# SIA-IDE/MMGT

Hardware: AMD Instinct MI355X
Metric: UNet3D denoise-steps/sec at 512x512x24 bf16 (higher is better)
Workload: dtype bf16; 1 GPU; BASELINE configs[1]: 512x512x24 pose2vid denoise step (CFG batch 2, UNet3D + MM-HAA, 16 reference banks, 1 window of 24 frames, guidance 3.5, DDIM v-pred), random-init weights; frames=24, parallelism=clip-parallel x1

## Files before the change

mmgt_amd/csrc/gemm.hip:

```cpp
#include <string.h>

#include <type_traits>

#include "common.h"
#include "gemm_common.h"
#include "mmgt_hip.h"

#ifndef MMGT_GEMM_VARIANT
#define MMGT_GEMM_VARIANT 7
#endif

namespace {

constexpr bool V_FRAGDB = (MMGT_GEMM_VARIANT & 1) != 0;
constexpr bool V_ILV = (MMGT_GEMM_VARIANT & 2) != 0;
constexpr bool V_LATE = (MMGT_GEMM_VARIANT & 4) != 0;
constexpr bool V_LATE_ALL = (MMGT_GEMM_VARIANT & 8) != 0;
constexpr bool V_NODMA = (MMGT_GEMM_VARIANT & 16) != 0;

template <int CTRL>
__device__ __forceinline__ unsigned dpp_quad(unsigned v) {
  return (unsigned)__builtin_amdgcn_mov_dpp((int)v, CTRL, 0xf, 0xf, true);
}
template <int S>
// ... 526 lines not shown
            }
          }
        };
        using std::integral_constant;
        group(integral_constant<int, 0>{}, integral_constant<int, (TN >= 2 ? 2 : 1)>{});
        if constexpr (TN > 2) group(integral_constant<int, 2>{}, integral_constant<int, (TN >= 4 ? 2 : 1)>{});
        if constexpr (TN > 4) group(integral_constant<int, 4>{}, integral_constant<int, (TN >= 6 ? 2 : 1)>{});
      }
    } else if (FULL_OK) {
#pragma unroll
      for (int i = 0; i < TM; ++i) {
        const int m = row0 + 32 * i + lr;
        if (m >= M) continue;
#pragma unroll
        for (int j = 0; j < TN; ++j) {
          if (geglu && (j & 1)) continue;
#pragma unroll
          for (int r = 0; r < 16; ++r) {
            const int nl = acc_row(r, lane);
            const int ncol = col0 + 32 * j + nl;
            if (ncol >= N) continue;
            float x = acc[i][j][r];
            if (ep.bias) x += ep.bias[ncol];
            long ocol = ncol;
            if (geglu) {
              float gte = acc[i][(j + 1) < TN ? j + 1 : j][r];
              if (ep.bias) gte += ep.bias[ncol + 32];
              x *= gelu_erf_f(gte);
              ocol = (long)((col0 + 32 * j) >> 1) + nl;
            } else {
              if (ep.bias2) x += ep.bias2[(long)(m / ep.bias2_rows) * N + ncol];
              if (ep.act == 2) x = silu_f(x);
              if (ep.act == 3) x = fmaxf(x, 0.f);
              if (ep.act == 4) x = quick_gelu_f(x);
              if (ep.act == 5) x = gelu_erf_f(x);
              if (ep.act == 6) x = mish_f(x);
              x *= (ep.row_scale ? ep.row_scale[m] : 1.f) * ep.alpha;
              if (POST_OK && ep.bias_post) x += ep.bias_post[ncol];
            }
            if (res) x += Elem<T>::ld(res + (long)m * ep.ldr + ocol);
            Elem<T>::st(out + (long)m * ep.ldo + ocol, x);
          }
        }
      }
    }
  }
}

template <typename T, int MODE, int BM, int BN, int WM, int WN, int NSTAGE, int ROWB = 128, int EPI = 0>
int launch_cfg(const ADesc& ad, const void* W, long bsw, const Epi& ep, int M, int N, int K, int batch, hipStream_t s) {
  const int tiles_m = (M + BM - 1) / BM, tiles_n = (N + BN - 1) / BN;
  const size_t lds = (size_t)NSTAGE * (BM + BN) * ROWB;
  auto kern = gemm_kernel<T, MODE, BM, BN, WM, WN, NSTAGE, ROWB, EPI>;
  static int resident = 0;
  if (!resident) {
    if (hipFuncSetAttribute(reinterpret_cast<const void*>(kern), hipFuncAttributeMaxDynamicSharedMemorySize, (int)lds) !=
        hipSuccess) {
      mmgt_set_error("gemm: cannot reserve %zu bytes of LDS", lds);
      return 2;
    }
    int per_cu = 0, dev = 0;
    hipDeviceProp_t prop;
    if (hipOccupancyMaxActiveBlocksPerMultiprocessor(&per_cu, kern, WM * WN * 64, lds) != hipSuccess || per_cu < 1 ||
        hipGetDevice(&dev) != hipSuccess || hipGetDeviceProperties(&prop, dev) != hipSuccess) {
      mmgt_set_error("gemm: occupancy query failed");
      return 2;
    }
    resident = per_cu * prop.multiProcessorCount;
  }
  long gx = (resident + batch - 1) / batch;
  gx = (gx + 7) / 8 * 8;
  if (gx > (long)tiles_m * tiles_n) gx = (long)tiles_m * tiles_n;
  dim3 grid((unsigned)gx, 1, batch);
  hipLaunchKernelGGL(kern, grid, dim3(WM * WN * 64), lds, s, ad, reinterpret_cast<const char*>(W), bsw, ep, M, N, K, tiles_m,
                     tiles_n);
  MMGT_LAUNCH_CHECK();
  return 0;
}

int g_splitk = 1;
int g_tailsplit = 1;
int g_gemm_cfg = 0;
int g_bm192 = 1;

}
int mmgt_gemm16_launch(int mode, int bn, const void* ad, const void* W, long bsw, const void* ep, int M, int N, int K,
                       int batch, void* stream);
int mmgt_gemm16_splitk(int mode, int bn, const void* ad, const void* W, const void* ep, int M, int N, int K, int S, void* stream, int m0);
namespace {

template <typename T, int MODE>
int launch(const ADesc& ad, const void* W, long bsw, const Epi& ep, int M, int N, int K, int batch, hipStream_t s) {
  const bool geglu = ep.act == 1;
  int cfg = g_gemm_cfg;
  if ((cfg == 0 || cfg == 18) && g_splitk && std::is_same<T, bf16_t>::value && batch == 1 && ep.act == 0 && ep.fast && !ep.row_scale &&
      ep.alpha == 1.f && !ep.bias_post && N % 8 == 0 && K >= 2560 && (N % 256 == 0 || N % 320 == 0) &&
      (((uintptr_t)ep.bias | (uintptr_t)ep.bias2) & 15) == 0) {
    const int bn = N % 256 == 0 ? 256 : 320;
    const long tiles = (long)((M + 255) / 256) * (N / bn);
    const int nch = K / 64;
    int S = 0;
    for (int c = 8; c >= 2; --c)
      if (tiles * c <= 256 && nch % c == 0 && nch / c >= (tiles <= 64 ? 16 : 64)) { S = c; break; }
    if (S >= 2 && tiles <= 128 && (MODE == 1 || tiles <= 32 || tiles > 64)) return mmgt_gemm16_splitk(MODE, bn, &ad, W, &ep, M, N, K, S, s, 0);
  }
  if (cfg == 18) cfg = 0;
  if (cfg == 0) {
    const long tiles128 = (long)((M + 127) / 128) * ((N + 127) / 128) * batch;
    const long tiles256 = (long)((M + 255) / 256) * ((N + 127) / 128) * batch;
    const long tiles256sq = (long)((M + 255) / 256) * ((N + 255) / 256) * batch;
    const bool big_ok = N % 256 == 0 && K >= 2560 && tiles256sq >= 192 && tiles256sq <= 512;
    const bool sq_ok = ((N + 255) / 256) * 256l * 100 <= (long)N * 107 && ((M + 255) / 256) * 256l * 100 <= (long)M * 115 && tiles256sq >= 192;
    const bool b16 = std::is_same<T, bf16_t>::value;
    if (MODE == 1) {
      if (b16 && N % 320 == 0 && (M >= 49152 || (M >= 24576 && N >= 640))) cfg = 17;
      else if (b16 && N % 256 == 0 && tiles256sq >= 192) cfg = 16;
      else cfg = (N % 320 == 0 && M >= 49152) ? 12 : big_ok ? 9 : (tiles128 < 512 || N <= 64) ? 3 : 1;
    } else if (b16 && !geglu && N % 320 == 0 && N <= 960 && M >= 131072) cfg = 17;
    else if (b16 && !geglu && N % 320 == 0 && N <= 1280 && M >= 49152 && (K >= 1280 || ep.residual || N == 1280)) cfg = 17;
    else if (b16 && !geglu && N == 640 && M >= 24576 && K >= 2560 && g_bm192) cfg = 17;
    else if (sq_ok) cfg = b16 ? 16 : 9;
    else if (geglu || K >= 1280) cfg = tiles256 >= 256 ? 6 : (!geglu && tiles128 <= 256) ? 3 : 1;
    else if (M >= 131072 && N >= 640) cfg = 6;
    else cfg = 1;
  }
  if (geglu && (cfg == 3 || cfg == 12)) cfg = 1;
  if (MODE == 1 && ad.up >= 2 && cfg != 16 && cfg != 17) cfg = N % 320 == 0 ? 17 : 16;
  bool bm192 = cfg == 19;
  if (cfg == 19) cfg = 17;
  if (cfg == 17 && !bm192 && g_gemm_cfg == 0 && g_bm192 && std::is_same<T, bf16_t>::value && batch == 1 && N % 320 == 0) {
    const long tn = N / 320;
    const long r256 = (((long)(M + 255) / 256) * tn + 255) / 256, r192 = (((long)(M + 191) / 192) * tn + 255) / 256;
    bm192 = (double)r192 * 0.88 < (double)r256 * 0.97;
  }
  if (cfg == 16 || cfg == 17) {
    const bool post = ep.row_scale || ep.alpha != 1.f || ep.bias_post;
    if (std::is_same<T, bf16_t>::value && ep.fast && ep.act <= (cfg == 16 && !post ? 1 : 0) &&
        (((uintptr_t)ep.bias | (uintptr_t)ep.bias2 | (uintptr_t)ep.bias_post) & 15) == 0 && N % 4 == 0) {
      const int bn = cfg == 16 ? 256 : bm192 ? 192320 : 320;
      const int bnc = cfg == 16 ? 256 : 320;
      const long tiles_n = (N + bnc - 1) / bnc, tiles_m = (M + 255) / 256, ntile = tiles_m * tiles_n;
      const int nch = K / 64;
      if (g_tailsplit && (!bm192 || g_gemm_cfg == 0) && MODE == 1 && batch == 1 && !ad.ksplit && ep.act == 0 && !post && N % bnc == 0 && N % 8 == 0 && K >= 2560 && nch % 2 == 0 && ntile > 256) {
        const long rows_a = (256 * (ntile / 256) / tiles_n) * 256;
        const long tail = (tiles_m - rows_a / 256) * tiles_n;
        const long img = MODE == 1 ? (long)ad.OH * ad.OW : 1;
        if (rows_a > 0 && rows_a < M && tail > 0 && 2 * tail <= 256 && 4 * tail >= 256 && rows_a % img == 0) {
          int rc = mmgt_gemm16_launch(MODE, bnc, &ad, W, bsw, &ep, (int)rows_a, N, K, 1, s);
          if (rc) return rc;
          ADesc adb = ad;
          Epi epb = ep;
          const long esz = sizeof(T);
          if (MODE == 1) {
            const long n0 = rows_a / img;
            adb.src0 = ad.src0 + n0 * ad.IH * ad.IW * ad.C0 * esz;
            if (ad.src1) adb.src1 = ad.src1 + n0 * ad.IH * ad.IW * ad.C1 * esz;
          } else {
            adb.src0 = ad.src0 + rows_a * ad.ld0 * esz;
          }
          if (ep.residual) epb.residual = ep.residual + rows_a * ep.ldr * esz;
          epb.out = ep.out + rows_a * ep.ldo * esz;
          return mmgt_gemm16_splitk(MODE, bnc, &adb, W, &epb, (int)(M - rows_a), N, K, 2, s, (int)rows_a);
        }
      }
      return mmgt_gemm16_launch(MODE, bn, &ad, W, bsw, &ep, M, N, K, batch, s);
    }
    if (MODE == 1 && ad.up >= 2) {
      mmgt_set_error("conv: the four-phase upsample form and the two-source 1 x 1 conv need the gemm16 path (bf16, 16-byte aligned bias, Cout %% 4 == 0)");
      return 1;
    }
    cfg = cfg == 16 ? 9 : geglu ? 1 : 12;
  }
  if (cfg == 20) {
    if (std::is_same<T, bf16_t>::value && ep.fast && ep.act == 0 && (((uintptr_t)ep.bias | (uintptr_t)ep.bias2 | (uintptr_t)ep.bias_post) & 15) == 0 && N % 4 == 0)
      return mmgt_gemm16_launch(MODE, 128, &ad, W, bsw, &ep, M, N, K, batch, s);
    cfg = 1;
  }
  if (!ep.fast || ep.act >= 2) return launch_cfg<T, MODE, 128, 128, 2, 2, 2, 128, 2>(ad, W, bsw, ep, M, N, K, batch, s);
  if (ep.row_scale || ep.alpha != 1.f || ep.bias_post) {
    if (MODE == 0 && !geglu) return launch_cfg<T, 0, 128, 128, 2, 2, 2, 128, 1>(ad, W, bsw, ep, M, N, K, batch, s);
    return launch_cfg<T, MODE, 128, 128, 2, 2, 2, 128, 2>(ad, W, bsw, ep, M, N, K, batch, s);
  }
#ifdef MMGT_GEMM_AB
  switch (cfg) {
    case 3: return launch_cfg<T, MODE, 128, 64, 2, 2, 2>(ad, W, bsw, ep, M, N, K, batch, s);
    case 6: return launch_cfg<T, MODE, 256, 128, 4, 2, 3>(ad, W, bsw, ep, M, N, K, batch, s);
    case 9: return launch_cfg<T, MODE, 256, 256, 2, 4, 2>(ad, W, bsw, ep, M, N, K, batch, s);
    case 12: return launch_cfg<T, MODE, 128, 320, 4, 2, 2>(ad, W, bsw, ep, M, N, K, batch, s);
    default: return launch_cfg<T, MODE, 128, 128, 2, 2, 2>(ad, W, bsw, ep, M, N, K, batch, s);
  }
#else
  switch (cfg) {
    case 1: return launch_cfg<T, MODE, 128, 128, 2, 2, 2>(ad, W, bsw, ep, M, N, K, batch, s);
    case 3: return launch_cfg<T, MODE, 128, 64, 2, 2, 2>(ad, W, bsw, ep, M, N, K, batch, s);
    case 6: return launch_cfg<T, MODE, 256, 128, 4, 2, 3>(ad, W, bsw, ep, M, N, K, batch, s);
    case 9: return launch_cfg<T, MODE, 256, 256, 2, 4, 2>(ad, W, bsw, ep, M, N, K, batch, s);
    case 12: return launch_cfg<T, MODE, 128, 320, 4, 2, 2>(ad, W, bsw, ep, M, N, K, batch, s);
    default: return launch_cfg<T, MODE, 128, 128, 2, 2, 2>(ad, W, bsw, ep, M, N, K, batch, s);
  }
#endif
}

int epi_fast(const Epi& ep, int N, int n_out, int esz) {
  auto al16 = [](const void* p) { return (reinterpret_cast<uintptr_t>(p) & 15) == 0; };
  bool ok = N % 8 == 0 && n_out % 8 == 0 && al16(ep.out) && (ep.ldo * esz) % 16 == 0 && (ep.bso * esz) % 16 == 0;
  ok = ok && (ep.bias2 == nullptr || ep.bias2_rows >= 256);
  if (ep.residual) ok = ok && al16(ep.residual) && (ep.ldr * esz) % 16 == 0 && (ep.bsr * esz) % 16 == 0;
  return ok ? 1 : 0;
}

int check_common(int dtype, int M, int N, int K, int act) {
  MMGT_CHECK(dtype == MMGT_F32 || dtype == MMGT_BF16, "gemm: bad dtype %d", dtype);
  MMGT_CHECK(M > 0 && N > 0 && K > 0, "gemm: empty problem M=%d N=%d K=%d", M, N, K);
  MMGT_CHECK(K % 64 == 0, "gemm: K=%d must be a multiple of 64 (pad channels on the host)", K);
  MMGT_CHECK(act >= 0 && act <= 6, "gemm: bad act %d", act);
  MMGT_CHECK(act != 1 || N % 64 == 0, "gemm: GEGLU needs N %% 64 == 0 (N=%d)", N);
  return 0;
}

}

void mmgt_attn_set64(int v);
void mmgt_gn_set_rows(int v);
void mmgt_attn_set_heads_inner(int v);
void mmgt_attn_set_attn80(int v);
void mmgt_attn_set_nomax(int v);
void mmgt_gemm16_set_pb(int v);
void mmgt_gemm16_set_stagger(int v);
void mmgt_gn_set_interleave(int v);
void mmgt_gn_set_lpr0(int v);
void mmgt_gn_set_narrow(int v);
void mmgt_gn_set_slab(int v);
void mmgt_ffn_set_dbg(int v);
void mmgt_rowgemm_set_dbg(int v);
void mmgt_tleg_set_abl(int v);
void mmgt_gnconv_set_abl(int v);
void mmgt_rconv_set_abl(int v);
void mmgt_rconv_set_stagger(int v);
void mmgt_rconv_set_cb(int v);
namespace {
struct HostSwitch { const char* key; int value; };
HostSwitch g_host[] = {
    {"fused_ff", 1},
    {"twin_attention", 1},
    {"shared_rows", 1},
    {"oz3", 1},
    {"rowgemm", 1},
    {"tleg", 1},
    {"rconv", 5},
    {"conv_out_taps", 1},
    {"ffpo_cat", 1},
    {"sc_cat", 1},
    {"up2", 1},
    {"rconv_stats", 1},
    {"gnconv", 2},
    {"zero_audio_skip", 1},
    {"window_state", 1},
    {"smga_graph", 1},
};
}
extern "C" int mmgt_tune_get(const char* key, int* value) {
  if (key && value)
    for (const HostSwitch& h : g_host)
      if (!strcmp(key, h.key)) { *value = h.value; return 0; }
  mmgt_set_error("tune_get: unknown key");
  return 1;
}
extern "C" int mmgt_tune(const char* key, int value) {
  if (key)
    for (HostSwitch& h : g_host)
      if (!strcmp(key, h.key)) { h.value = value; return 0; }
  if (key && !strcmp(key, "gemm_cfg")) { g_gemm_cfg = value; return 0; }
  if (key && !strcmp(key, "attn64")) { mmgt_attn_set64(value); return 0; }
  if (key && !strcmp(key, "attn_nomax") && (value == 0 || value == 1)) { mmgt_attn_set_nomax(value); return 0; }
  if (key && !strcmp(key, "attn_heads_inner")) { mmgt_attn_set_heads_inner(value); return 0; }
  if (key && !strcmp(key, "attn80")) { mmgt_attn_set_attn80(value); return 0; }
  if (key && !strcmp(key, "g16_pb")) { mmgt_gemm16_set_pb(value); return 0; }
  if (key && !strcmp(key, "g16_stagger")) { mmgt_gemm16_set_stagger(value); return 0; }
  if (key && !strcmp(key, "gn_rows")) { mmgt_gn_set_rows(value); return 0; }
  if (key && !strcmp(key, "gn_interleave")) { mmgt_gn_set_interleave(value); return 0; }
  if (key && !strcmp(key, "gn_narrow")) { mmgt_gn_set_narrow(value); return 0; }
  if (key && !strcmp(key, "gn_slab")) { mmgt_gn_set_slab(value); return 0; }
  if (key && !strcmp(key, "gn_lpr0")) { if (value != 4 && value != 8 && value != 16) return -1; mmgt_gn_set_lpr0(value); return 0; }
  if (key && !strcmp(key, "splitk")) { g_splitk = value; return 0; }
  if (key && !strcmp(key, "bm192")) { g_bm192 = value; return 0; }
  if (key && !strcmp(key, "tailsplit")) { g_tailsplit = value; return 0; }
  if (key && !strcmp(key, "rconv_cb") && (value == 0 || value == 320 || value == 256 || value == 160)) { mmgt_rconv_set_cb(value); return 0; }
  if (key && !strcmp(key, "rconv_stagger") && value >= 0 && value <= 8192) { mmgt_rconv_set_stagger(value); return 0; }
#ifdef MMGT_ABLATE
  if (key && !strcmp(key, "ffn_dbg") && value >= 0 && value <= 2) { mmgt_ffn_set_dbg(value); return 0; }
  if (key && !strcmp(key, "gnconv_abl") && value >= 0 && value <= 255) { mmgt_gnconv_set_abl(value); return 0; }
  if (key && !strcmp(key, "tleg_abl") && value >= 0 && value <= 128) { mmgt_tleg_set_abl(value); return 0; }
  if (key && !strcmp(key, "rconv_abl") && value >= 0 && value <= 31) { mmgt_rconv_set_abl(value); return 0; }
  if (key && !strcmp(key, "rowgemm_dbg") && value >= 0 && value <= 5) { mmgt_rowgemm_set_dbg(value); return 0; }
#else
  if (key && !strcmp(key, "rowgemm_dbg") && (value == 0 || value == 5)) { mmgt_rowgemm_set_dbg(value); return 0; }
  if (key && (!strcmp(key, "ffn_dbg") || !strcmp(key, "gnconv_abl") || !strcmp(key, "tleg_abl") || !strcmp(key, "rconv_abl") || !strcmp(key, "rowgemm_dbg"))) {
    mmgt_set_error("tune: '%s' selects a timing ablation whose results are garbage; the product library does not contain them (build libmmgt_hip_abl.so with `make -C mmgt_amd/csrc abl` and load it through MMGT_LIB)", key);
    return 1;
  }
#endif
  mmgt_set_error("tune: unknown key");
  return 1;
}

namespace {
template <typename T>
__global__ __launch_bounds__(256) void gemv_kernel(const T* __restrict__ A, long lda, const T* __restrict__ W, const float* __restrict__ bias,
                                                   T* __restrict__ out, long ldo, int M, int N, int K, int act) {
  constexpr int VEC = 16 / sizeof(T);
  const int lane = threadIdx.x & 63, n = blockIdx.x * 4 + (threadIdx.x >> 6);
  if (n >= N) return;
  float acc[4] = {0.f, 0.f, 0.f, 0.f};
  const T* w = W + (long)n * K;
  for (int k = lane * VEC; k < K; k += 64 * VEC) {
    union { u32x4 u; T e[VEC]; } wv, av;
    wv.u = *reinterpret_cast<const u32x4*>(w + k);
#pragma unroll
    for (int m = 0; m < 4; ++m)
      if (m < M) {
        av.u = *reinterpret_cast<const u32x4*>(A + m * lda + k);
#pragma unroll
        for (int e = 0; e < VEC; ++e) acc[m] = fmaf(Elem<T>::ld(&wv.e[e]), Elem<T>::ld(&av.e[e]), acc[m]);
      }
  }
#pragma unroll
  for (int m = 0; m < 4; ++m) {
    float v = acc[m];
    for (int o = 32; o > 0; o >>= 1) v += __shfl_xor(v, o);
    if (lane == 0 && m < M) {
      v += bias ? bias[n] : 0.f;
      if (act == 2) v = silu_f(v);
      Elem<T>::st(out + m * ldo + n, v);
    }
  }
}
}

static int gemm_entry(const void* A, long lda, const void* W, const float* bias, const float* bias2, int bias2_rows,
                      const float* row_scale, float alpha, const float* bias_post, const void* residual, long ldr, void* out,
                      long ldo, int M, int N, int K, int act, int batch, long bsA, long bsW, long bsR, long bsO, int dtype,
                      void* stream) {
  if (check_common(dtype, M, N, K, act)) return 1;
  MMGT_CHECK(A && W && out, "gemm: null pointer");
  MMGT_CHECK(lda >= 1 && batch >= 1, "gemm: lda %ld < 1 or batch %d < 1", lda, batch);
  MMGT_CHECK(!bias2 || bias2_rows > 0, "gemm: bias2_rows must be positive");
  const int esz = dtype == MMGT_BF16 ? 2 : 4;
  MMGT_CHECK(((uintptr_t)A % 16) == 0 && ((uintptr_t)W % 16) == 0 && (lda * esz) % 16 == 0 && (bsA * esz) % 16 == 0 &&
                 (bsW * esz) % 16 == 0,
             "gemm: A/W must be 16-byte aligned with 16-byte aligned rows");
  MMGT_CHECK(((long)(M - 1) * lda + K) * esz < (1l << 31) && (long)N * K * esz < (1l << 31),
             "gemm: an operand (per batch entry) exceeds the 2 GiB range of the 32-bit LDS-DMA offsets");
  if (M == 1 && batch == 1 && !bias2 && !row_scale && alpha == 1.f && !bias_post && !residual && (act == 0 || act == 2) && K % (16 / esz) == 0) {
    if (dtype == MMGT_BF16)
      hipLaunchKernelGGL(gemv_kernel<bf16_t>, dim3((unsigned)((N + 3) / 4)), dim3(256), 0, (hipStream_t)stream, (const bf16_t*)A, lda, (const bf16_t*)W, bias,
                         (bf16_t*)out, ldo, M, N, K, act);
    else
      hipLaunchKernelGGL(gemv_kernel<float>, dim3((unsigned)((N + 3) / 4)), dim3(256), 0, (hipStream_t)stream, (const float*)A, lda, (const float*)W, bias,
                         (float*)out, ldo, M, N, K, act);
    MMGT_LAUNCH_CHECK();
    return 0;
  }
  ADesc ad{};
  ad.src0 = (const char*)A;
  ad.ld0 = lda;
  ad.bs0 = bsA;
  Epi ep{};
  ep.bias = bias; ep.bias2 = bias2; ep.bias2_rows = bias2_rows; ep.row_scale = row_scale; ep.alpha = alpha;
// ... 89 lines not shown
```

mmgt_amd/csrc/gemm16.hip:

```cpp
#include <type_traits>

#include "common.h"
#include "gemm_common.h"
#include "mmgt_hip.h"

namespace {

typedef __attribute__((ext_vector_type(4))) float acc4;

__device__ __forceinline__ acc4 mma16(s16x8 a, s16x8 b, acc4 c) {
  return __builtin_amdgcn_mfma_f32_16x16x32_bf16(a, b, c, 0, 0, 0);
}

template <int MODE, int BN, int BM = 256>
__global__ __launch_bounds__(512, 2) void gemm16_kernel(ADesc ad, const char* __restrict__ W, long bsw, Epi ep, int M, int N,
                                                        int K, int tiles_m, int tiles_n, int pb_stg, unsigned long long* trace) {
  extern __shared__ __attribute__((aligned(1024))) char smem[];
  typedef bf16_t T;
  static_assert(BN == 128 || BN == 256 || BN == 320, "BN");
  static_assert(BM == 256 || BM == 192, "BM");
  constexpr int ESZ = 2, ROWB = 128, BK = 64, NW = 8;
  constexpr int WROWS = BM / 4, RT = WROWS / 16;
  constexpr int A_BYTES = BM * ROWB, B_BYTES = BN * ROWB, STAGE_BYTES = A_BYTES + B_BYTES;
  constexpr int CPR = 8, RPD = 8;
  constexpr int GA = BM / RPD / NW, GB = BN / RPD / NW;
  constexpr int NPH = BN / 64, NT = BN / 32;
  constexpr int BIAS_OFF = 2 * STAGE_BYTES, BIAS_ARR = 2048, NBP = BN == 320 ? 2 : 1;
  auto swz = [](int row) { return (row >> 1) & 7; };

  const int nwg = tiles_m * tiles_n;
  const int pb = pb_stg & 255, stg = pb_stg >> 8;
  const int bz = blockIdx.z;
  const int tid = threadIdx.x, lane = tid & 63, wid = __builtin_amdgcn_readfirstlane(tid >> 6);
  const int wr = wid >> 2;
  const int wm = wid >> 1, wn = wid & 1;
  const int lm = lane & 15, lq = lane >> 4;
  int trace_n = 0;
  auto stamp = [&](int k) {
    if (trace && (wid & 3) == 0 && lane == 0 && trace_n < 32) trace[(((long)blockIdx.x * 32 + trace_n) * 2 + wr) * 4 + k] = wall_clock64();
  };

  auto decode = [&](int v, int& tm, int& tn) {
    const int q = nwg >> 3, r = nwg & 7, x = v & 7;
    const int t = (x < r ? x * (q + 1) : r * (q + 1) + (x - r) * q) + (v >> 3);
    if (pb <= 1) {
      tm = t / tiles_n;
      tn = t - tm * tiles_n;
    } else {
      const int gsz = pb * tiles_n, g = t / gsz, w = t - g * gsz;
      const int pbe = min(pb, tiles_m - g * pb);
      tn = w / pbe;
      tm = g * pb + (w - tn * pbe);
    }
  };

  const int srow = lane / CPR, spos = lane % CPR;
  const int ldw = ad.ksplit ? ad.ldw : K;
  const long kstart = ad.ksplit ? (long)bz * K : 0;
  const T* a0 = reinterpret_cast<const T*>(ad.src0) + (ad.ksplit ? (MODE == 0 ? kstart : 0) : (long)bz * ad.bs0);
  const T* a1 = ad.src1 ? reinterpret_cast<const T*>(ad.src1) + (ad.ksplit ? 0 : (long)bz * ad.bs1) : nullptr;
  const T* wbase = reinterpret_cast<const T*>(W) + (ad.ksplit ? kstart : (long)bz * bsw);
  const __amdgpu_buffer_rsrc_t rA0 = dma_rsrc(a0), rA1 = dma_rsrc(a1 ? a1 : a0), rW = dma_rsrc(wbase);
  const int c0sw = spos ^ (srow >> 1);
  int limA = 0, limW = 0;
  unsigned aoff[MODE == 0 ? 2 : GA];
  unsigned woff[2];
  unsigned am0 = 0;
  int a_step = 0, w_step = 0;
  int p_tap = 0, p_c = 0, a_soff = 0;
  bool a_second = false, a_fresh = true;
  auto setupA = [&](int tm) {
    const unsigned row = (unsigned)(tm * BM + wid * GA * RPD + srow);
    if (MODE == 0) {
      a_step = (int)(RPD * ad.ld0 * ESZ);
      limA = M - (int)row;
#pragma unroll
      for (int q = 0; q < 2; ++q) aoff[q] = row * (unsigned)(ad.ld0 * ESZ) + (unsigned)((c0sw ^ (4 * ((q + wid * GA) & 1))) << 4);
    } else {
      am0 = row;
    }
    p_tap = MODE == 1 ? (int)(kstart / (ad.C0 + ad.C1)) : 0;
    p_c = MODE == 1 ? (int)(kstart - (long)p_tap * (ad.C0 + ad.C1)) : 0;
    a_fresh = true;
  };
  auto setupW = [&](int tn) {
    const unsigned row = (unsigned)(tn * BN + wid * GB * RPD + srow);
    w_step = RPD * ldw * ESZ;
    limW = N - (int)row;
#pragma unroll
    for (int q = 0; q < 2; ++q) woff[q] = row * (unsigned)(ldw * ESZ) + (unsigned)((c0sw ^ (4 * ((q + wid * GB) & 1))) << 4);
  };
  auto prepA = [&](int ch) {
    if (MODE == 0) {
      a_soff = ch * ROWB;
    } else {
      const int cin = ad.C0 + ad.C1;
      if (p_c == 0 || p_c == ad.C0 || a_fresh) {
        a_fresh = false;
        const bool up2 = ad.up == 2;
        const int ky = up2 ? p_tap >> 1 : ad.up == 3 ? 1 : p_tap / 3, kx = up2 ? p_tap & 1 : ad.up == 3 ? 1 : p_tap - ky * 3;
        const int vh = ad.up == 1 ? ad.IH * 2 : ad.IH, vw = ad.up == 1 ? ad.IW * 2 : ad.IW;
        const bool second = p_c >= ad.C0 && ad.C1 > 0;
        const unsigned cpb = (unsigned)(second ? ad.C1 : ad.C0) * ESZ;
        a_second = second;
        a_soff = (p_c - (second ? ad.C0 : 0)) * ESZ;
// ... 135 lines not shown
        int m = row0 + 16 * i + lm;
        if (m >= M) m = M - 1;
        second[i] = ep.bias2 && m / b2div != b2r0;
      }
#pragma unroll
      for (int j = 0; j < NT; ++j) {
        const acc4 b = ep.bias ? lb[4 * j] : (acc4)(0.f);
        if (ep.bias2) {
          const acc4 r0v = lb[BIAS_ARR / 16 + 4 * j], r1v = lb[2 * BIAS_ARR / 16 + 4 * j];
#pragma unroll
          for (int i = 0; i < RT; ++i) acc[i][j] = b + (second[i] ? r1v : r0v);
        } else {
#pragma unroll
          for (int i = 0; i < RT; ++i) acc[i][j] = b;
        }
      }
    } else {
#pragma unroll
      for (int i = 0; i < RT; ++i)
#pragma unroll
        for (int j = 0; j < NT; ++j) acc[i][j] = (acc4)(0.f);
    }

    stamp(0);
    s16x8 fa[RT][2], fb[2][2];
    for (int ch = 0; ch < nchunks; ++ch) {
      if (trace && (wid & 3) == 0 && lane == 0 && trace_n < 8 && ch < 16)
        trace[65536 + (((long)blockIdx.x * 8 + trace_n) * 2 + wr) * 16 + ch] = wall_clock64();
      const char* st = smem + sc * STAGE_BYTES;
      const bool skipW = w_pre && ch == 0;
      const bool moreW = !skipW && giW < total, moreA = giA < total;
      const int stW = giW & 1, stA = giA & 1, chW = ichW;
      if (moreA) prepA(ichA);
      for_n(integral_constant<int, NPH>{}, [&](auto Pc) {
        constexpr int P = decltype(Pc)::value;
#pragma unroll
        for (int t = 0; t < 2; ++t) {
          const char* pb = st + b_base + (32 * P + 16 * t) * ROWB;
          fb[t][0] = *reinterpret_cast<const s16x8*>(pb + roff0);
          fb[t][1] = *reinterpret_cast<const s16x8*>(pb + roff1);
        }
        if (P == 0) {
#pragma unroll
          for (int t = 0; t < RT; ++t) {
            const char* pa = st + a_base + 16 * t * ROWB;
            fa[t][0] = *reinterpret_cast<const s16x8*>(pa + roff0);
            fa[t][1] = *reinterpret_cast<const s16x8*>(pa + roff1);
          }
        }
        if (P == 1 && ch == 0 && wr == 0 && (ep.bias_post || (has_bias && vt + G < nwg))) issue_bias(has_bias && vt + G < nwg ? vt + G : -1, vt);
        constexpr int PLO = BN == 128 ? (P == 0 ? 0 : GB) : 2 * P, PN = BN == 128 ? (P == 0 ? GB : GA) : 2;
        for_n(integral_constant<int, PN>{}, [&](auto Uc) {
          constexpr int S = PLO + decltype(Uc)::value;
          if constexpr (S < GB) {
            if (moreW) issueW(stW, chW, integral_constant<int, S>{});
            if constexpr (S == GB - 1) { if (moreW) advanceW(); }
          } else if constexpr (S < GB + GA) {
            if (moreA) issueA(stA, integral_constant<int, S - GB>{});
            if constexpr (S == GB + GA - 1) { if (moreA) advanceA(); }
          }
        });
        if (P == NPH - 1) {
          constexpr int NST = RT * (NT / 2);
          if (skipW && w_relax) {
            if (ep.act == 1) { if (moreA) wait_vmcnt<GA + NST / 2>(); else wait_vmcnt<NST / 2>(); }
            else { if (moreA) wait_vmcnt<GA + NST>(); else wait_vmcnt<NST>(); }
          } else {
            if (moreA) wait_vmcnt<GA>(); else wait_vmcnt<0>();
          }
        }
        asm volatile("s_waitcnt lgkmcnt(0)" ::: "memory");
        __builtin_amdgcn_sched_barrier(0);
        __builtin_amdgcn_s_barrier();
        __builtin_amdgcn_sched_barrier(0);
        __builtin_amdgcn_s_setprio(1);
#pragma unroll
        for (int ks = 0; ks < 2; ++ks)
#pragma unroll
          for (int t = 0; t < RT; ++t)
#pragma unroll
            for (int u = 0; u < 2; ++u) acc[t][2 * P + u] = mma16(fb[u][ks], fa[t][ks], acc[t][2 * P + u]);
        __builtin_amdgcn_s_setprio(0);
        __builtin_amdgcn_sched_barrier(0);
        if (!(P == NPH - 1 && wr == 1 && ch == nchunks - 1)) __builtin_amdgcn_s_barrier();
        __builtin_amdgcn_sched_barrier(0);
      });
      sc ^= 1;
    }

    w_pre = giW < total;
    if (w_pre) {
      for_n(integral_constant<int, GB>{}, [&](auto i) { issueW(giW & 1, ichW, i); });
      advanceW();
    }
    w_relax = !ad.ksplit && nchunks >= 2 && tm * BM + BM <= M && tn * BN + BN <= N;
    int lme = lm, lqe = lq;
    asm volatile("" : "+v"(lme), "+v"(lqe));
    stamp(1);
    constexpr int NPAIR = NT / 2;
    stamp(2);
    auto epilogue = [&](auto Gc, auto Rc, auto Pc) {
      constexpr bool GEGLU = decltype(Gc)::value, RES = decltype(Rc)::value, POST = decltype(Pc)::value;
      constexpr int NBUF = (BN == 256 || (MODE == 0 && !POST)) ? 2 : 1;
      const int cofs = 16 * (lqe & 1) + 8 * (lqe >> 1);
      const int ncol = N - (col0 + cofs);
      T* obase = reinterpret_cast<T*>(ep.out) + (long)bz * ep.bso + (GEGLU ? (col0 >> 1) + cofs : col0 + cofs);
      const T* rbase = RES ? reinterpret_cast<const T*>(ep.residual) + (long)bz * ep.bsr + col0 + cofs : nullptr;
      u32x4 rv[RES ? NBUF : 1][RES ? NPAIR : 1];
      auto load_res = [&](int i, u32x4* dst) {
        const int m = row0 + 16 * i + lme;
        const T* rrow = rbase + (long)(m < M ? m : M - 1) * ep.ldr;
#pragma unroll
        for (int jp = 0; jp < NPAIR; ++jp) dst[jp] = *reinterpret_cast<const u32x4*>(rrow + (32 * jp < ncol ? 32 * jp : ncol - 8));
      };
      if (RES && NBUF == 2) load_res(0, rv[0]);
      float rsv[POST ? RT : 1];
      const acc4* lpost = reinterpret_cast<const acc4*>(smem + BIAS_OFF + 3 * BIAS_ARR) + ((wn * (BN / 2) + cofs) >> 2);
      if (POST) {
#pragma unroll
        for (int i = 0; i < RT; ++i) {
          const int m = row0 + 16 * i + lme;
          rsv[i] = (ep.row_scale ? ep.row_scale[m < M ? m : M - 1] : 1.f) * ep.alpha;
        }
      }
#pragma unroll
      for (int i = 0; i < RT; ++i) {
        const int m = row0 + 16 * i + lme;
        T* orow = obase + (long)m * ep.ldo;
        if (MODE == 1 && ad.up == 2) {
          const unsigned mm = (unsigned)(m < M ? m : M - 1);
          const unsigned cn = fastdiv(mm, ad.fd_hw), rem = mm - cn * (unsigned)(ad.OH * ad.OW);
          const unsigned oy = fastdiv(rem, ad.fd_ow), ox = rem - oy * (unsigned)ad.OW;
          orow = obase + ((long)(cn * 2u * (unsigned)ad.OH + 2u * oy + (unsigned)(bz >> 1)) * (2 * ad.OW) + 2 * ox + (bz & 1)) * ep.ldo;
        }
        if (RES) {
          if (NBUF == 2 ? i < RT - 1 : true) load_res(NBUF == 2 ? i + 1 : i, rv[NBUF == 2 ? (i + 1) & 1 : 0]);
        }
#pragma unroll
        for (int jp = 0; jp < NPAIR; ++jp) {
          if (GEGLU && (jp & 1)) continue;
          acc4 x = acc[i][2 * jp], y = acc[i][2 * jp + 1];
          if (GEGLU) {
            const acc4 gx = acc[i][(2 * jp + 2) % NT], gy = acc[i][(2 * jp + 3) % NT];
            const f32x2 g0 = gelu_erf_f2((f32x2){gx[0], gx[1]}), g1 = gelu_erf_f2((f32x2){gx[2], gx[3]});
            const f32x2 g2 = gelu_erf_f2((f32x2){gy[0], gy[1]}), g3 = gelu_erf_f2((f32x2){gy[2], gy[3]});
            x[0] *= g0[0]; x[1] *= g0[1]; x[2] *= g1[0]; x[3] *= g1[1];
            y[0] *= g2[0]; y[1] *= g2[1]; y[2] *= g3[0]; y[3] *= g3[1];
          }
          if (!RES && !POST) {
            const auto s01 = __builtin_amdgcn_permlane16_swap(pack_bf16x2(x[0], x[1]), pack_bf16x2(y[0], y[1]), false, false);
            const auto s23 = __builtin_amdgcn_permlane16_swap(pack_bf16x2(x[2], x[3]), pack_bf16x2(y[2], y[3]), false, false);
            if (m < M && 32 * jp < ncol)
              st_out16(orow + (GEGLU ? 16 * jp : 32 * jp), (u32x4){s01[0], s23[0], s01[1], s23[1]});
            continue;
          }
          float o8[8];
#pragma unroll
          for (int r = 0; r < 4; ++r) {
            const auto sw2 = __builtin_amdgcn_permlane16_swap(__float_as_uint(x[r]), __float_as_uint(y[r]), false, false);
            o8[r] = __uint_as_float(sw2[0]);
            o8[4 + r] = __uint_as_float(sw2[1]);
          }
          if (POST) {
            const acc4 pa = ep.bias_post ? lpost[8 * jp] : (acc4)(0.f), pb = ep.bias_post ? lpost[8 * jp + 1] : (acc4)(0.f);
#pragma unroll
            for (int e = 0; e < 4; ++e) {
              o8[e] = fmaf(o8[e], rsv[i], pa[e]);
              o8[4 + e] = fmaf(o8[4 + e], rsv[i], pb[e]);
            }
          }
          if (RES) {
            union { u32x4 u; bf16_t e[8]; } r8;
            r8.u = rv[NBUF == 2 ? i & 1 : 0][jp];
#pragma unroll
            for (int e = 0; e < 8; ++e) o8[e] += bf16_to_f32(r8.e[e]);
          }
          if (m < M && 32 * jp < ncol)
            st_out16(orow + (GEGLU ? 16 * jp : 32 * jp),
                     (u32x4){pack_bf16x2(o8[0], o8[1]), pack_bf16x2(o8[2], o8[3]), pack_bf16x2(o8[4], o8[5]), pack_bf16x2(o8[6], o8[7])});
        }
      }
    };
    using std::true_type;
    using std::false_type;
    const bool post = ep.row_scale != nullptr || ep.alpha != 1.f || ep.bias_post != nullptr;
    if (ad.ksplit) {
      float* pb = reinterpret_cast<float*>(ep.out) + (long)bz * ep.bso + col0 + 4 * lqe;
#pragma unroll
      for (int i = 0; i < RT; ++i) {
        const int m = row0 + 16 * i + lme;
#pragma unroll
        for (int j = 0; j < NT; ++j)
          if (m < M && col0 + 16 * j + 4 * lqe < N) *reinterpret_cast<acc4*>(pb + (long)m * ep.ldo + 16 * j) = acc[i][j];
      }
    } else if (BN == 256 && ep.act == 1) {
      if constexpr (BN == 256) {
        if (ep.residual) epilogue(true_type{}, true_type{}, false_type{}); else epilogue(true_type{}, false_type{}, false_type{});
      }
    } else if (post) {
      if (ep.residual) epilogue(false_type{}, true_type{}, true_type{}); else epilogue(false_type{}, false_type{}, true_type{});
    } else if (ep.residual) {
      epilogue(false_type{}, true_type{}, false_type{});
    } else {
      epilogue(false_type{}, false_type{}, false_type{});
    }
    stamp(3);
    ++trace_n;
    if (wr == 1) __builtin_amdgcn_s_barrier();
  }
  if (wr == 0) __builtin_amdgcn_s_barrier();
}

unsigned long long* g_trace = nullptr;
int g_stg = -1;
int g_pb = -1;

template <int MODE, int BN, int BM = 256>
int launch16(const ADesc& ad, const void* W, long bsw, const Epi& ep, int M, int N, int K, int batch, hipStream_t s) {
  const int tiles_m = (M + BM - 1) / BM, tiles_n = (N + BN - 1) / BN;
  const size_t lds = (size_t)2 * (BM + BN) * 128 + 4 * 2048;
  auto kern = gemm16_kernel<MODE, BN, BM>;
  static int resident = 0;
  if (!resident) {
    if (hipFuncSetAttribute(reinterpret_cast<const void*>(kern), hipFuncAttributeMaxDynamicSharedMemorySize, (int)lds) !=
        hipSuccess) {
      mmgt_set_error("gemm16: cannot reserve %zu bytes of LDS", lds);
      return 2;
    }
    int dev = 0;
    hipDeviceProp_t prop;
    if (hipGetDevice(&dev) != hipSuccess || hipGetDeviceProperties(&prop, dev) != hipSuccess) {
      mmgt_set_error("gemm16: device query failed");
      return 2;
    }
    resident = prop.multiProcessorCount;
  }
  long gx = (resident + batch - 1) / batch;
  gx = (gx + 7) / 8 * 8;
  if (gx > (long)tiles_m * tiles_n) gx = (long)tiles_m * tiles_n;
  dim3 grid((unsigned)gx, 1, batch);
  const int pb = g_pb >= 0 ? g_pb : (MODE == 0 && tiles_n >= 8 && tiles_m >= 8) ? 8 : 1;
  const int stg = g_stg >= 0 ? g_stg : (MODE == 0 && ep.residual && !ad.ksplit && K <= 1280) ? 10 : 0;
  hipLaunchKernelGGL(kern, grid, dim3(512), lds, s, ad, reinterpret_cast<const char*>(W), bsw, ep, M, N, K, tiles_m, tiles_n, pb | (stg << 8), g_trace);
  MMGT_LAUNCH_CHECK();
  return 0;
}

}

extern "C" void mmgt_gemm16_set_trace(void* p) { g_trace = reinterpret_cast<unsigned long long*>(p); }
void mmgt_gemm16_set_pb(int v) { g_pb = v; }
void mmgt_gemm16_set_stagger(int v) { g_stg = v; }

namespace {

__global__ __launch_bounds__(256) void splitk_reduce_kernel(const float* __restrict__ part, int S, long slab, const float* __restrict__ bias,
                                                            const float* __restrict__ bias2, int b2rows, const bf16_t* __restrict__ res,
                                                            long ldr, bf16_t* __restrict__ out, long ldo, int M, int N, int m0) {
  const int nv = N / 8;
  const long idx = (long)blockIdx.x * 256 + threadIdx.x;
  if (idx >= (long)M * nv) return;
  const int m = (int)(idx / nv), c = (int)(idx - (long)m * nv) * 8;
  const float* p = part + (long)m * N + c;
  f32x4 a0 = *reinterpret_cast<const f32x4*>(p), a1 = *reinterpret_cast<const f32x4*>(p + 4);
  for (int z = 1; z < S; ++z) {
    a0 += *reinterpret_cast<const f32x4*>(p + z * slab);
    a1 += *reinterpret_cast<const f32x4*>(p + z * slab + 4);
  }
  if (bias) { a0 += *reinterpret_cast<const f32x4*>(bias + c); a1 += *reinterpret_cast<const f32x4*>(bias + c + 4); }
  if (bias2) {
    const float* b2 = bias2 + (long)((m + m0) / b2rows) * N + c;
    a0 += *reinterpret_cast<const f32x4*>(b2);
    a1 += *reinterpret_cast<const f32x4*>(b2 + 4);
  }
  if (res) {
    union { u32x4 u; bf16_t e[8]; } r8;
    r8.u = *reinterpret_cast<const u32x4*>(res + (long)m * ldr + c);
#pragma unroll
    for (int e = 0; e < 4; ++e) { a0[e] += bf16_to_f32(r8.e[e]); a1[e] += bf16_to_f32(r8.e[4 + e]); }
  }
  *reinterpret_cast<u32x4*>(out + (long)m * ldo + c) =
      (u32x4){pack_bf16x2(a0[0], a0[1]), pack_bf16x2(a0[2], a0[3]), pack_bf16x2(a1[0], a1[1]), pack_bf16x2(a1[2], a1[3])};
}

constexpr int MAX_DEV = 16, MAX_RETIRED = 8;
struct SplitkWs {
  float* p = nullptr; size_t bytes = 0; bool captured = false;
  float* retired[MAX_RETIRED] = {};
  size_t retired_bytes[MAX_RETIRED] = {};
  int nretired = 0;
};
SplitkWs g_splitk_ws[MAX_DEV];

float* splitk_workspace(size_t need, hipStream_t s) {
  int dev = 0;
  if (hipGetDevice(&dev) != hipSuccess || dev < 0 || dev >= MAX_DEV) {
    mmgt_set_error("gemm16 split-K: device query failed");
    return nullptr;
  }
  SplitkWs& w = g_splitk_ws[dev];
  hipStreamCaptureStatus cs = hipStreamCaptureStatusNone;
  const bool capturing = hipStreamIsCapturing(s, &cs) == hipSuccess && cs != hipStreamCaptureStatusNone;
  if (need > w.bytes) {
    if (capturing) {
      mmgt_set_error("gemm16 split-K: the partial-sum workspace would have to grow to %zu bytes inside a stream capture; run the "
                     "shape once outside the capture (warm-up) first", need);
      return nullptr;
    }
    size_t want = need;
    if (w.bytes && want < 2 * w.bytes) want = 2 * w.bytes;
    if (w.p && !w.captured) {
      (void)hipFree(w.p);
    } else if (w.p) {
      if (w.nretired == MAX_RETIRED) {
        mmgt_set_error("gemm16 split-K: %d captured workspaces already retired; destroy the graphs that hold them and restart", MAX_RETIRED);
        return nullptr;
      }
      w.retired[w.nretired] = w.p;
      w.retired_bytes[w.nretired++] = w.bytes;
    }
    w.p = nullptr; w.bytes = 0; w.captured = false;
    if (hipMalloc(reinterpret_cast<void**>(&w.p), want) != hipSuccess) {
      if (want == need || hipMalloc(reinterpret_cast<void**>(&w.p), need) != hipSuccess) {
        w.p = nullptr;
        mmgt_set_error("gemm16 split-K: cannot allocate %zu bytes of partial sums", need);
        return nullptr;
      }
      want = need;
    }
    w.bytes = want;
  }
  if (capturing) w.captured = true;
  return w.p;
}

}

int mmgt_gemm16_splitk(int mode, int bn, const void* adp, const void* W, const void* epp, int M, int N, int K, int S, void* stream, int m0) {
  ADesc ad = *reinterpret_cast<const ADesc*>(adp);
  const Epi& ep = *reinterpret_cast<const Epi*>(epp);
  hipStream_t s = (hipStream_t)stream;
  const size_t need = (size_t)S * M * N * sizeof(float);
  float* ws = splitk_workspace(need, s);
  if (!ws) return 2;
  ad.ksplit = 1;
  ad.ldw = K;
  Epi pe{};
  pe.out = reinterpret_cast<char*>(ws);
  pe.ldo = N;
  pe.bso = (long)M * N;
  pe.alpha = 1.f;
  pe.fast = 1;
  const int ks = K / S;
  int rc;
  if (bn == 320) rc = mode == 0 ? launch16<0, 320>(ad, W, 0, pe, M, N, ks, S, s) : launch16<1, 320>(ad, W, 0, pe, M, N, ks, S, s);
  else rc = mode == 0 ? launch16<0, 256>(ad, W, 0, pe, M, N, ks, S, s) : launch16<1, 256>(ad, W, 0, pe, M, N, ks, S, s);
  if (rc) return rc;
  const long nthr = (long)M * (N / 8);
  hipLaunchKernelGGL(splitk_reduce_kernel, dim3((unsigned)((nthr + 255) / 256)), dim3(256), 0, s, ws, S, (long)M * N, ep.bias, ep.bias2,
                     ep.bias2 ? ep.bias2_rows : 1, reinterpret_cast<const bf16_t*>(ep.residual), ep.ldr, reinterpret_cast<bf16_t*>(ep.out), ep.ldo, M, N, m0);
  MMGT_LAUNCH_CHECK();
  return 0;
}

extern "C" int mmgt_gemm_bf16_f32(const void* A, long lda, const void* W, long ldw, float* out, long ldo, int M, int N, int K, void* stream) {
  MMGT_CHECK(A && W && out && M > 0 && N > 0 && K > 0, "gemm_bf16_f32: bad arguments");
  MMGT_CHECK(K % 64 == 0 && N % 8 == 0 && lda >= K && ldw >= K && ldo >= N && lda % 8 == 0 && ldw % 8 == 0 && ldo % 4 == 0,
             "gemm_bf16_f32: unsupported shape M=%d N=%d K=%d lda=%ld ldw=%ld ldo=%ld", M, N, K, lda, ldw, ldo);
  MMGT_CHECK(((uintptr_t)A % 16) == 0 && ((uintptr_t)W % 16) == 0 && ((uintptr_t)out % 16) == 0, "gemm_bf16_f32: pointers must be 16-byte aligned");
  MMGT_CHECK(((long)(M - 1) * lda + K) * 2 < (1l << 31) && ((long)(N - 1) * ldw + K) * 2 < (1l << 31),
             "gemm_bf16_f32: an operand exceeds the 2 GiB range of the 32-bit LDS-DMA offsets");
  ADesc ad{};
  ad.src0 = reinterpret_cast<const char*>(A);
  ad.ld0 = lda;
  ad.ksplit = 1;
  ad.ldw = (int)ldw;
  Epi pe{};
  pe.out = reinterpret_cast<char*>(out);
  pe.ldo = ldo;
  pe.alpha = 1.f;
  pe.fast = 1;
  return launch16<0, 256>(ad, W, 0, pe, M, N, K, 1, (hipStream_t)stream);
}

int mmgt_gemm16_launch(int mode, int bn, const void* adp, const void* W, long bsw, const void* epp, int M, int N, int K,
                       int batch, void* stream) {
  const ADesc& ad = *reinterpret_cast<const ADesc*>(adp);
  const Epi& ep = *reinterpret_cast<const Epi*>(epp);
  hipStream_t s = (hipStream_t)stream;
  if (bn == 192320) return mode == 0 ? launch16<0, 320, 192>(ad, W, bsw, ep, M, N, K, batch, s) : launch16<1, 320, 192>(ad, W, bsw, ep, M, N, K, batch, s);
  if (bn == 320) return mode == 0 ? launch16<0, 320>(ad, W, bsw, ep, M, N, K, batch, s) : launch16<1, 320>(ad, W, bsw, ep, M, N, K, batch, s);
  if (bn == 128) return mode == 0 ? launch16<0, 128>(ad, W, bsw, ep, M, N, K, batch, s) : launch16<1, 128>(ad, W, bsw, ep, M, N, K, batch, s);
  return mode == 0 ? launch16<0, 256>(ad, W, bsw, ep, M, N, K, batch, s) : launch16<1, 256>(ad, W, bsw, ep, M, N, K, batch, s);
}
```

Baseline: 14.75 steps/s.

## Add small-tile two-workgroup-per-CU gemm16 variants for small upsampled-conv GEMMs

Adds 128x128 and 64x128 tile variants of the gemm16 kernel that run 4 waves (256 threads) per workgroup, skip the ping-pong inter-wave barriers, and size the persistent grid for two resident workgroups per CU. The heuristic routes bf16 implicit-conv GEMMs with up==3 and M between 2048 and 4096, K<=2560 to the 64x128 variant. The aim is more parallel tiles and better CU fill on small-M GEMMs where 256-row tiles leave most CUs idle. The trade-off is lower per-tile data reuse and losing the wave ping-pong schedule on those shapes.

```diff
diff --git a/mmgt_amd/csrc/gemm.hip b/mmgt_amd/csrc/gemm.hip
--- a/mmgt_amd/csrc/gemm.hip
+++ b/mmgt_amd/csrc/gemm.hip
@@ -632,6 +632,7 @@
 int g_tailsplit = 1;
 int g_gemm_cfg = 0;
 int g_bm192 = 1;
+int g_2wg = 1;
 
 }
 int mmgt_gemm16_launch(int mode, int bn, const void* ad, const void* W, long bsw, const void* ep, int M, int N, int K,
@@ -639,10 +640,17 @@
 int mmgt_gemm16_splitk(int mode, int bn, const void* ad, const void* W, const void* ep, int M, int N, int K, int S, void* stream, int m0);
 namespace {
 
+int pick_2wg(const ADesc& ad, const Epi& ep, int mode, int M, int N, int K, int batch) {
+  if (batch != 1 || ep.act != 0 || !ep.fast || N % 128 != 0) return 0;
+  if (mode == 1 && ad.up == 3 && M >= 2048 && M <= 4096 && K <= 2560) return 22;
+  return 0;
+}
+
 template <typename T, int MODE>
 int launch(const ADesc& ad, const void* W, long bsw, const Epi& ep, int M, int N, int K, int batch, hipStream_t s) {
   const bool geglu = ep.act == 1;
   int cfg = g_gemm_cfg;
+  if (cfg == 0 && g_2wg && std::is_same<T, bf16_t>::value) cfg = pick_2wg(ad, ep, MODE, M, N, K, batch);
   if ((cfg == 0 || cfg == 18) && g_splitk && std::is_same<T, bf16_t>::value && batch == 1 && ep.act == 0 && ep.fast && !ep.row_scale &&
       ep.alpha == 1.f && !ep.bias_post && N % 8 == 0 && K >= 2560 && (N % 256 == 0 || N % 320 == 0) &&
       (((uintptr_t)ep.bias | (uintptr_t)ep.bias2) & 15) == 0) {
@@ -675,7 +683,13 @@
     else cfg = 1;
   }
   if (geglu && (cfg == 3 || cfg == 12)) cfg = 1;
-  if (MODE == 1 && ad.up >= 2 && cfg != 16 && cfg != 17) cfg = N % 320 == 0 ? 17 : 16;
+  if (MODE == 1 && ad.up >= 2 && cfg != 16 && cfg != 17 && !(ad.up == 3 && (cfg == 21 || cfg == 22))) cfg = N % 320 == 0 ? 17 : 16;
+  if (cfg == 21 || cfg == 22) {
+    if (std::is_same<T, bf16_t>::value && ep.fast && ep.act == 0 && (((uintptr_t)ep.bias | (uintptr_t)ep.bias2 | (uintptr_t)ep.bias_post) & 15) == 0 &&
+        N % 4 == 0 && !(MODE == 1 && ad.up == 2))
+      return mmgt_gemm16_launch(MODE, cfg == 21 ? 128128 : 64128, &ad, W, bsw, &ep, M, N, K, batch, s);
+    cfg = MODE == 1 && ad.up >= 2 ? (N % 320 == 0 ? 17 : 16) : 1;
+  }
   bool bm192 = cfg == 19;
   if (cfg == 19) cfg = 17;
   if (cfg == 17 && !bm192 && g_gemm_cfg == 0 && g_bm192 && std::is_same<T, bf16_t>::value && batch == 1 && N % 320 == 0) {
@@ -834,6 +848,7 @@
   if (key && !strcmp(key, "gn_lpr0")) { if (value != 4 && value != 8 && value != 16) return -1; mmgt_gn_set_lpr0(value); return 0; }
   if (key && !strcmp(key, "splitk")) { g_splitk = value; return 0; }
   if (key && !strcmp(key, "bm192")) { g_bm192 = value; return 0; }
+  if (key && !strcmp(key, "g16_2wg")) { g_2wg = value; return 0; }
   if (key && !strcmp(key, "tailsplit")) { g_tailsplit = value; return 0; }
   if (key && !strcmp(key, "rconv_cb") && (value == 0 || value == 320 || value == 256 || value == 160)) { mmgt_rconv_set_cb(value); return 0; }
   if (key && !strcmp(key, "rconv_stagger") && value >= 0 && value <= 8192) { mmgt_rconv_set_stagger(value); return 0; }
diff --git a/mmgt_amd/csrc/gemm16.hip b/mmgt_amd/csrc/gemm16.hip
--- a/mmgt_amd/csrc/gemm16.hip
+++ b/mmgt_amd/csrc/gemm16.hip
@@ -13,14 +13,15 @@
 }
 
 template <int MODE, int BN, int BM = 256>
-__global__ __launch_bounds__(512, 2) void gemm16_kernel(ADesc ad, const char* __restrict__ W, long bsw, Epi ep, int M, int N,
+__global__ __launch_bounds__(BM <= 128 ? 256 : 512, 2) void gemm16_kernel(ADesc ad, const char* __restrict__ W, long bsw, Epi ep, int M, int N,
                                                         int K, int tiles_m, int tiles_n, int pb_stg, unsigned long long* trace) {
   extern __shared__ __attribute__((aligned(1024))) char smem[];
   typedef bf16_t T;
   static_assert(BN == 128 || BN == 256 || BN == 320, "BN");
-  static_assert(BM == 256 || BM == 192, "BM");
-  constexpr int ESZ = 2, ROWB = 128, BK = 64, NW = 8;
-  constexpr int WROWS = BM / 4, RT = WROWS / 16;
+  static_assert(BM == 256 || BM == 192 || ((BM == 128 || BM == 64) && BN == 128), "BM");
+  constexpr int ESZ = 2, ROWB = 128, BK = 64, NW = BM <= 128 ? 4 : 8;
+  constexpr bool PP = NW == 8;
+  constexpr int WROWS = BM / (NW / 2), RT = WROWS / 16;
   constexpr int A_BYTES = BM * ROWB, B_BYTES = BN * ROWB, STAGE_BYTES = A_BYTES + B_BYTES;
   constexpr int CPR = 8, RPD = 8;
   constexpr int GA = BM / RPD / NW, GB = BN / RPD / NW;
@@ -322,7 +323,7 @@
             for (int u = 0; u < 2; ++u) acc[t][2 * P + u] = mma16(fb[u][ks], fa[t][ks], acc[t][2 * P + u]);
         __builtin_amdgcn_s_setprio(0);
         __builtin_amdgcn_sched_barrier(0);
-        if (!(P == NPH - 1 && wr == 1 && ch == nchunks - 1)) __builtin_amdgcn_s_barrier();
+        if (PP && !(P == NPH - 1 && wr == 1 && ch == nchunks - 1)) __builtin_amdgcn_s_barrier();
         __builtin_amdgcn_sched_barrier(0);
       });
       sc ^= 1;
@@ -448,7 +449,7 @@
     ++trace_n;
     if (wr == 1) __builtin_amdgcn_s_barrier();
   }
-  if (wr == 0) __builtin_amdgcn_s_barrier();
+  if (PP && wr == 0) __builtin_amdgcn_s_barrier();
 }
 
 unsigned long long* g_trace = nullptr;
@@ -459,6 +460,7 @@
 int launch16(const ADesc& ad, const void* W, long bsw, const Epi& ep, int M, int N, int K, int batch, hipStream_t s) {
   const int tiles_m = (M + BM - 1) / BM, tiles_n = (N + BN - 1) / BN;
   const size_t lds = (size_t)2 * (BM + BN) * 128 + 4 * 2048;
+  constexpr int NTHR = BM <= 128 ? 256 : 512;
   auto kern = gemm16_kernel<MODE, BN, BM>;
   static int resident = 0;
   if (!resident) {
@@ -467,21 +469,26 @@
       mmgt_set_error("gemm16: cannot reserve %zu bytes of LDS", lds);
       return 2;
     }
-    int dev = 0;
+    int per_cu = 0, dev = 0;
     hipDeviceProp_t prop;
-    if (hipGetDevice(&dev) != hipSuccess || hipGetDeviceProperties(&prop, dev) != hipSuccess) {
+    if (hipOccupancyMaxActiveBlocksPerMultiprocessor(&per_cu, kern, NTHR, lds) != hipSuccess || per_cu < 1 ||
+        hipGetDevice(&dev) != hipSuccess || hipGetDeviceProperties(&prop, dev) != hipSuccess) {
       mmgt_set_error("gemm16: device query failed");
       return 2;
     }
-    resident = prop.multiProcessorCount;
+    if (BM <= 128 && per_cu < 2) {
+      mmgt_set_error("gemm16: the %d x %d tile holds %d workgroup(s) per CU, not 2", BM, BN, per_cu);
+      return 2;
+    }
+    resident = (BM <= 128 ? 2 : 1) * prop.multiProcessorCount;
   }
   long gx = (resident + batch - 1) / batch;
   gx = (gx + 7) / 8 * 8;
   if (gx > (long)tiles_m * tiles_n) gx = (long)tiles_m * tiles_n;
   dim3 grid((unsigned)gx, 1, batch);
   const int pb = g_pb >= 0 ? g_pb : (MODE == 0 && tiles_n >= 8 && tiles_m >= 8) ? 8 : 1;
-  const int stg = g_stg >= 0 ? g_stg : (MODE == 0 && ep.residual && !ad.ksplit && K <= 1280) ? 10 : 0;
-  hipLaunchKernelGGL(kern, grid, dim3(512), lds, s, ad, reinterpret_cast<const char*>(W), bsw, ep, M, N, K, tiles_m, tiles_n, pb | (stg << 8), g_trace);
+  const int stg = BM <= 128 ? 0 : g_stg >= 0 ? g_stg : (MODE == 0 && ep.residual && !ad.ksplit && K <= 1280) ? 10 : 0;
+  hipLaunchKernelGGL(kern, grid, dim3(NTHR), lds, s, ad, reinterpret_cast<const char*>(W), bsw, ep, M, N, K, tiles_m, tiles_n, pb | (stg << 8), g_trace);
   MMGT_LAUNCH_CHECK();
   return 0;
 }
@@ -630,6 +637,8 @@
   hipStream_t s = (hipStream_t)stream;
   if (bn == 192320) return mode == 0 ? launch16<0, 320, 192>(ad, W, bsw, ep, M, N, K, batch, s) : launch16<1, 320, 192>(ad, W, bsw, ep, M, N, K, batch, s);
   if (bn == 320) return mode == 0 ? launch16<0, 320>(ad, W, bsw, ep, M, N, K, batch, s) : launch16<1, 320>(ad, W, bsw, ep, M, N, K, batch, s);
+  if (bn == 128128) return mode == 0 ? launch16<0, 128, 128>(ad, W, bsw, ep, M, N, K, batch, s) : launch16<1, 128, 128>(ad, W, bsw, ep, M, N, K, batch, s);
+  if (bn == 64128) return mode == 0 ? launch16<0, 128, 64>(ad, W, bsw, ep, M, N, K, batch, s) : launch16<1, 128, 64>(ad, W, bsw, ep, M, N, K, batch, s);
   if (bn == 128) return mode == 0 ? launch16<0, 128>(ad, W, bsw, ep, M, N, K, batch, s) : launch16<1, 128>(ad, W, bsw, ep, M, N, K, batch, s);
   return mode == 0 ? launch16<0, 256>(ad, W, bsw, ep, M, N, K, batch, s) : launch16<1, 256>(ad, W, bsw, ep, M, N, K, batch, s);
 }
```

After: 14.67 steps/s (median of 2 runs). No clear change (-0.5%).
